# jyegerlehner/tensorflow-wavenet

Measured on AMD Instinct MI355X. Metric: audio samples/sec (train, default wavenet_params.json), higher is better.
Workload: dtype f32

## Files before the change

tensorflow-wavenet_amd/csrc/wn_gemm.hip:

```cpp
#include "wn_common.h"
#include <cstdlib>
#include <cstddef>
#include <cstring>

struct GemmNN {
  const float* A;
  long lda;
  long a_plane_stride;
  int a_planes;
  const float* W;
  int ldw;
  const float* bias;
  const float* mask;
  long ld_mask;
  const float* addend;
  long ld_add;
  float* C;
  long ldc;
  long c_plane_stride;
  int c_planes;
  float* Cpre;
  long M;
  int N, K;
  int relu;
// ... 162 lines not shown
        v[q] = *reinterpret_cast<const f32x4*>(tile + row * EP_LD + cc);
        if (g.mask && ok)
          mk[q] = __builtin_bit_cast(f32x4, __builtin_amdgcn_raw_buffer_load_b128(rM, vM, it * sM, EP_LD_AUX));
        if (g.addend && ok)
          ad[q] = __builtin_bit_cast(f32x4, __builtin_amdgcn_raw_buffer_load_b128(rA, vA, it * sA, EP_LD_AUX));
      }
#pragma unroll
      for (int q = 0; q < 4; ++q) {
        const int it = bt * 4 + q, row = it * 4 + rr;
        if (!(ncol && row < nrows)) continue;
        f32x4 x = v[q] + bias4;
        if (g.Cpre)
          __builtin_amdgcn_raw_buffer_store_b128(__builtin_bit_cast(ep_u32x4, x), rP, vP, it * sP, EP_ST_AUX);
        if (g.relu) {
#pragma unroll
          for (int e = 0; e < 4; ++e) x[e] = fmaxf(x[e], 0.f);
        }
        if (g.mask) {
#pragma unroll
          for (int e = 0; e < 4; ++e) x[e] = mk[q][e] > 0.f ? x[e] : 0.f;
        }
        if (g.addend) x += ad[q];
        __builtin_amdgcn_raw_buffer_store_b128(__builtin_bit_cast(ep_u32x4, x), rC, vC, it * sC, EP_ST_AUX);
      }
    }
  }
  }
}

template <int WMT>
__global__ __launch_bounds__(WMT * 128) void gemm_nn_kernel(GemmNN g) {
  constexpr int TM = WMT * 64, NT = WMT * 128;
  constexpr int NA = TM * 8 / NT, NB = 1024 / NT;
  __shared__ __attribute__((aligned(16))) float smem[2 * TM * NN_KC + 2 * NN_KC * NN_TN];
  float (*As)[TM * NN_KC] = reinterpret_cast<float (*)[TM * NN_KC]>(smem);
  float (*Bs)[NN_KC * NN_TN] =
      reinterpret_cast<float (*)[NN_KC * NN_TN]>(smem + 2 * TM * NN_KC);
  static_assert(WMT * 2 * 32 * EP_LD <= 2 * TM * NN_KC + 2 * NN_KC * NN_TN, "epilogue LDS");
  const int tid = threadIdx.x, lane = tid & 63, wave = tid >> 6;
  const int j = lane & 31, h = lane >> 5;
  const int wm = wave % WMT, wn = wave / WMT;
  const int logical = xcd_remap(blockIdx.x, g.nwg);
  const int tile_n = logical % g.tiles_n;
  const long m0 = (long)(logical / g.tiles_n) * TM;
  const int n0 = tile_n * NN_TN;
  const int nk = (g.K + NN_KC - 1) / NN_KC;
  f32x4 ra[NA], rb[NB];
  const bool full_m = m0 + TM <= g.M, full_n = n0 + NN_TN <= g.N;
  auto gload = [&](int kc) {
    const bool full_k = (kc + 1) * NN_KC <= g.K;
    if (full_m && full_k) {
      const float* pa = g.a_planes
                            ? g.A + (long)kc * g.a_plane_stride + m0 * 32
                            : g.A + m0 * g.lda + kc * NN_KC;
      const long ld = g.a_planes ? 32 : g.lda;
#pragma unroll
      for (int i = 0; i < NA; ++i)
        ra[i] = *reinterpret_cast<const f32x4*>(
            pa + (long)((tid >> 3) + (NT / 8) * i) * ld + (tid & 7) * 4);
    } else {
#pragma unroll
      for (int i = 0; i < NA; ++i) {
        const int row = (tid >> 3) + (NT / 8) * i, ch = tid & 7;
        const long m = m0 + row;
        const int k = kc * NN_KC + ch * 4;
        f32x4 v = {0.f, 0.f, 0.f, 0.f};
        if (m < g.M && k < g.K) {
          const float* p = g.a_planes
                               ? g.A + (long)kc * g.a_plane_stride + m * 32 + ch * 4
                               : g.A + m * g.lda + k;
          v = *reinterpret_cast<const f32x4*>(p);
        }
        ra[i] = v;
      }
    }
    if (full_n && full_k) {
      const float* pb = g.W + (long)kc * NN_KC * g.ldw + n0;
#pragma unroll
      for (int i = 0; i < NB; ++i)
        rb[i] = *reinterpret_cast<const f32x4*>(
            pb + (long)((tid >> 5) + (NT / 32) * i) * g.ldw + (tid & 31) * 4);
    } else {
#pragma unroll
      for (int i = 0; i < NB; ++i) {
        const int kk = (tid >> 5) + (NT / 32) * i, c4 = tid & 31;
        const int k = kc * NN_KC + kk, n = n0 + c4 * 4;
        f32x4 v = {0.f, 0.f, 0.f, 0.f};
        if (k < g.K && n < g.N)
          v = *reinterpret_cast<const f32x4*>(g.W + (long)k * g.ldw + n);
        rb[i] = v;
      }
    }
  };
  auto sstore = [&](int buf) {
#pragma unroll
    for (int i = 0; i < NA; ++i) {
      const int row = (tid >> 3) + (NT / 8) * i, ch = tid & 7;
      const int sw = ch ^ ((row >> 1) & 7);
      *reinterpret_cast<f32x4*>(&As[buf][row * NN_KC + sw * 4]) = ra[i];
    }
#pragma unroll
    for (int i = 0; i < NB; ++i) {
      const int kk = (tid >> 5) + (NT / 32) * i, c4 = tid & 31;
      *reinterpret_cast<f32x4*>(&Bs[buf][kk * NN_TN + c4 * 4]) = rb[i];
    }
  };

  f32x16 acc[2][2];
#pragma unroll
  for (int a = 0; a < 2; ++a)
#pragma unroll
    for (int b = 0; b < 2; ++b) acc[a][b] = frag_zero();

  gload(0);
  sstore(0);
  __syncthreads();
  for (int kc = 0; kc < nk; ++kc) {
    const int buf = kc & 1;
    if (kc + 1 < nk) gload(kc + 1);
    f32x16 fa[2];
#pragma unroll
    for (int fm = 0; fm < 2; ++fm) {
      const int row = wm * 64 + fm * 32 + j;
#pragma unroll
      for (int q = 0; q < 4; ++q) {
        const int sw = (2 * q + h) ^ ((j >> 1) & 7);
        const f32x4 v =
            *reinterpret_cast<const f32x4*>(&As[buf][row * NN_KC + sw * 4]);
        fa[fm][4 * q + 0] = v[0];
        fa[fm][4 * q + 1] = v[1];
        fa[fm][4 * q + 2] = v[2];
        fa[fm][4 * q + 3] = v[3];
      }
    }
    const float* bl = &Bs[buf][4 * h * NN_TN + wn * 64 + j];
#pragma unroll
    for (int r = 0; r < 16; ++r) {
      const int ko = (8 * (r >> 2) + (r & 3)) * NN_TN;
      const float w0 = bl[ko], w1 = bl[ko + 32];
      acc[0][0] = __builtin_amdgcn_mfma_f32_32x32x2f32(w0, fa[0][r], acc[0][0], 0, 0, 0);
      acc[0][1] = __builtin_amdgcn_mfma_f32_32x32x2f32(w0, fa[1][r], acc[0][1], 0, 0, 0);
      acc[1][0] = __builtin_amdgcn_mfma_f32_32x32x2f32(w1, fa[0][r], acc[1][0], 0, 0, 0);
      acc[1][1] = __builtin_amdgcn_mfma_f32_32x32x2f32(w1, fa[1][r], acc[1][1], 0, 0, 0);
    }
    if (kc + 1 < nk) sstore(buf ^ 1);
    __syncthreads();
  }

  gemm_epilogue(g, acc, smem, m0, n0, wm, wn, wave, lane);
}

#define N3_KC 16
#define N3_STAGE (NN_TM * N3_KC + N3_KC * NN_TN)

typedef __bf16 bf16x8 __attribute__((ext_vector_type(8)));
typedef unsigned int u32x4 __attribute__((ext_vector_type(4)));

struct Split3 {
  bf16x8 p[3];
};

__device__ __forceinline__ Split3 split3(const float (&v)[8]) {
  unsigned int hi[8], mi[8], lo[8];
#pragma unroll
  for (int e = 0; e < 8; ++e) {
    const unsigned int u = __float_as_uint(v[e]) & 0xffff0000u;
    const float r = v[e] - __uint_as_float(u);
    const unsigned int m = __float_as_uint(r) & 0xffff0000u;
    const float r2 = r - __uint_as_float(m);
    hi[e] = u;
    mi[e] = m;
    lo[e] = __float_as_uint(r2);
  }
  Split3 s;
  u32x4 ph, pm, pl;
#pragma unroll
  for (int w = 0; w < 4; ++w) {
    ph[w] = __builtin_amdgcn_perm(hi[2 * w + 1], hi[2 * w], 0x07060302u);
    pm[w] = __builtin_amdgcn_perm(mi[2 * w + 1], mi[2 * w], 0x07060302u);
    pl[w] = __builtin_amdgcn_perm(lo[2 * w + 1], lo[2 * w], 0x07060302u);
  }
  s.p[0] = __builtin_bit_cast(bf16x8, ph);
  s.p[1] = __builtin_bit_cast(bf16x8, pm);
  s.p[2] = __builtin_bit_cast(bf16x8, pl);
  return s;
}

template <int NPROD>
__device__ __forceinline__ void mma_split(f32x16& acc, const Split3& a, const Split3& b) {
#define WN_MM(i, k) \
  acc = __builtin_amdgcn_mfma_f32_32x32x16_bf16(a.p[i], b.p[k], acc, 0, 0, 0)
  if (NPROD >= 9) { WN_MM(2, 2); WN_MM(1, 2); WN_MM(2, 1); }
  if (NPROD >= 6) { WN_MM(1, 1); WN_MM(0, 2); WN_MM(2, 0); }
  WN_MM(0, 1);
  WN_MM(1, 0);
  WN_MM(0, 0);
#undef WN_MM
}

template <bool STAMPS>
__device__ __forceinline__ void nn3_tile(const GemmNN& g, float* smem, int tile_n, long m0,
                                         long m_end, unsigned long long* dbg) {
#define NSTAMP(i) if (STAMPS && threadIdx.x == 0) dbg[i] = __builtin_amdgcn_s_memtime()
  const int tid = threadIdx.x, lane = tid & 63;
  const int wave = __builtin_amdgcn_readfirstlane(tid >> 6);
  const int j = lane & 31, h = lane >> 5;
  const int wm = wave & 1, wn = wave >> 1;
  const int n0 = tile_n * NN_TN;
  const int nk = g.K / N3_KC;
  const bool live = n0 + wn * 64 < g.N;

  const int a_slot = lane & 3;
  const int a_chunk = a_slot ^ ((lane >> 4) & 3);
  long am0 = m0 + 16 * wave + (lane >> 2), am1 = am0 + 64;
  am0 = am0 < g.M ? am0 : g.M - 1;
  am1 = am1 < g.M ? am1 : g.M - 1;
  const long lda = g.a_planes ? 32 : g.lda;
  const int va0 = (int)((am0 * lda + a_chunk * 4) * 4);
  const int va1 = (int)((am1 * lda + a_chunk * 4) * 4);
  int wcol = n0 + (lane & 31) * 4;
  wcol = wcol < g.N ? wcol : 0;
  const int vw0 = (int)(((long)(2 * wave + (lane >> 5)) * g.ldw + wcol) * 4);
  const int vw1 = vw0 + (int)(8L * g.ldw * 4);
  auto stage = [&](int kc, float* base) {
    const __amdgpu_buffer_rsrc_t rsA = ep_rsrc(
        g.A + (g.a_planes ? (long)(kc >> 1) * g.a_plane_stride + (kc & 1) * 16 : (long)kc * N3_KC));
    const __amdgpu_buffer_rsrc_t rsW = ep_rsrc(g.W + (long)kc * N3_KC * g.ldw);
    __builtin_amdgcn_raw_ptr_buffer_load_lds(rsA, (lptr_t)(base + wave * 256), 16, va0, 0, 0, 0);
    __builtin_amdgcn_raw_ptr_buffer_load_lds(rsA, (lptr_t)(base + (wave + 4) * 256), 16, va1, 0, 0, 0);
    float* wb = base + NN_TM * N3_KC;
    __builtin_amdgcn_raw_ptr_buffer_load_lds(rsW, (lptr_t)(wb + wave * 256), 16, vw0, 0, 0, 0);
    __builtin_amdgcn_raw_ptr_buffer_load_lds(rsW, (lptr_t)(wb + (wave + 4) * 256), 16, vw1, 0, 0, 0);
  };

  f32x16 acc[2][2];
#pragma unroll
  for (int a = 0; a < 2; ++a)
#pragma unroll
    for (int b = 0; b < 2; ++b) acc[a][b] = frag_zero();

  stage(0, smem);
  if (!live) {
    for (int kc = 0; kc < nk; ++kc) {
      asm volatile("s_waitcnt vmcnt(0)\n\ts_barrier" ::: "memory");
      if (kc + 1 < nk) stage(kc + 1, smem + ((kc & 1) ^ 1) * N3_STAGE);
    }
  }
  for (int kc = 0; live && kc < nk; ++kc) {
    const int ST = kc & 1;
    asm volatile("s_waitcnt vmcnt(0)\n\ts_barrier" ::: "memory");
    if (STAMPS && kc == 0) { NSTAMP(1); }
    if (kc + 1 < nk) stage(kc + 1, smem + (ST ^ 1) * N3_STAGE);
    const float* As = smem + ST * N3_STAGE;
    const float* Bs = As + NN_TM * N3_KC;
    f32x4 fa[2][2];
#pragma unroll
    for (int fm = 0; fm < 2; ++fm) {
      const int row = wm * 64 + fm * 32 + j;
#pragma unroll
      for (int q = 0; q < 2; ++q)
        fa[fm][q] = *reinterpret_cast<const f32x4*>(
            As + row * N3_KC + (((2 * q + h) ^ ((row >> 2) & 3)) << 2));
    }
    const float* bl = Bs + 4 * h * NN_TN + wn * 64 + j;
    __builtin_amdgcn_s_setprio(1);
    constexpr int PF = NN3_PF;
    float wv[8][2];
#pragma unroll
    for (int r = 0; r < PF; ++r) {
      const int ko = (8 * (r >> 2) + (r & 3)) * NN_TN;
      wv[r][0] = bl[ko];
      wv[r][1] = bl[ko + 32];
    }
    __builtin_amdgcn_sched_barrier(0);
#pragma unroll
    for (int r = 0; r < 8; ++r) {
      if (r + PF < 8) {
        const int ko = (8 * ((r + PF) >> 2) + ((r + PF) & 3)) * NN_TN;
        wv[r + PF][0] = bl[ko];
        wv[r + PF][1] = bl[ko + 32];
      }
      __builtin_amdgcn_sched_barrier(0);
      const float w0 = wv[r][0], w1 = wv[r][1];
      const float x0 = fa[0][r >> 2][r & 3], x1 = fa[1][r >> 2][r & 3];
      acc[0][0] = __builtin_amdgcn_mfma_f32_32x32x2f32(w0, x0, acc[0][0], 0, 0, 0);
      acc[0][1] = __builtin_amdgcn_mfma_f32_32x32x2f32(w0, x1, acc[0][1], 0, 0, 0);
      acc[1][0] = __builtin_amdgcn_mfma_f32_32x32x2f32(w1, x0, acc[1][0], 0, 0, 0);
      acc[1][1] = __builtin_amdgcn_mfma_f32_32x32x2f32(w1, x1, acc[1][1], 0, 0, 0);
      __builtin_amdgcn_sched_barrier(0);
    }
    __builtin_amdgcn_s_setprio(0);
  }
  NSTAMP(2);
  asm volatile("s_waitcnt lgkmcnt(0)\n\ts_barrier" ::: "memory");
  NSTAMP(3);
  gemm_epilogue(g, acc, smem, m0, n0, wm, wn, wave, lane, m_end);
  NSTAMP(4);
#undef NSTAMP
}

constexpr int NN3_LDSF = 2 * N3_STAGE > 4 * 32 * EP_LD ? 2 * N3_STAGE : 4 * 32 * EP_LD;

__global__ __launch_bounds__(256, 4) void gemm_nn3_kernel(GemmNN g) {
  __shared__ __attribute__((aligned(1024))) float smem[NN3_LDSF];
  unsigned long long* dbg = nullptr;
#ifdef NN3_STAMPS
// ... 341 lines not shown
  __shared__ __attribute__((aligned(16))) float As[32 * TM];
  __shared__ __attribute__((aligned(16))) float Gs[32 * TNW];
  const int tid = threadIdx.x, lane = tid & 63, wave = tid >> 6;
  const int i = lane & 31, h = lane >> 5;
  const int tn = blockIdx.x % g.tiles_n, tm = blockIdx.x / g.tiles_n;
  const int m0 = tm * TM, n0 = tn * TNW;
  const long r_begin = (long)blockIdx.y * g.rows_per_split;
  long r_end = r_begin + g.rows_per_split;
  if (r_end > g.rows) r_end = g.rows;

  f32x16 acc[MF][NF];
#pragma unroll
  for (int a = 0; a < MF; ++a)
#pragma unroll
    for (int b = 0; b < NF; ++b) acc[a][b] = frag_zero();
  float cs[NF];
#pragma unroll
  for (int b = 0; b < NF; ++b) cs[b] = 0.f;

  f32x4 ra[NA], rg[NG];
  auto gload = [&](long r0) {
#pragma unroll
    for (int k = 0; k < NA; ++k) {
      const int idx = tid + 256 * k;
      f32x4 v = {0.f, 0.f, 0.f, 0.f};
      if (idx < 32 * A4) {
        const int row = idx / A4, c4 = idx - row * A4;
        const long r = r0 + row;
        if (r < r_end) {
          const int m = m0 + c4 * 4;
          const float* p = g.a_planes
                               ? g.A + (long)(m >> 5) * g.a_plane_stride + r * 32 + (m & 31)
                               : g.A + r * g.lda + m;
          v = *reinterpret_cast<const f32x4*>(p);
        }
      }
      ra[k] = v;
    }
#pragma unroll
    for (int k = 0; k < NG; ++k) {
      const int idx = tid + 256 * k;
      const int row = idx / G4, c4 = idx - row * G4;
      const long r = r0 + row;
      f32x4 v = {0.f, 0.f, 0.f, 0.f};
      if (r < r_end)
        v = *reinterpret_cast<const f32x4*>(g.G + r * g.ldg + n0 + c4 * 4);
      rg[k] = v;
    }
  };
  auto sstore = [&]() {
#pragma unroll
    for (int k = 0; k < NA; ++k) {
      const int idx = tid + 256 * k;
      if (idx < 32 * A4) *reinterpret_cast<f32x4*>(&As[idx * 4]) = ra[k];
    }
#pragma unroll
    for (int k = 0; k < NG; ++k)
      *reinterpret_cast<f32x4*>(&Gs[(tid + 256 * k) * 4]) = rg[k];
  };

  gload(r_begin);
  sstore();
  __syncthreads();
  for (long r0 = r_begin; r0 < r_end; r0 += 32) {
    const bool more = r0 + 32 < r_end;
    if (more) gload(r0 + 32);
    const float* al = As + h * TM + i;
    const float* gl = Gs + h * TNW + wave * (NF * 32) + i;
#pragma unroll 2
    for (int s = 0; s < 16; ++s) {
      float av[MF], bv[NF];
#pragma unroll
      for (int a = 0; a < MF; ++a) av[a] = al[2 * s * TM + a * 32];
#pragma unroll
      for (int b = 0; b < NF; ++b) {
        bv[b] = gl[2 * s * TNW + b * 32];
        cs[b] += bv[b];
      }
#pragma unroll
      for (int a = 0; a < MF; ++a)
#pragma unroll
        for (int b = 0; b < NF; ++b)
          acc[a][b] = __builtin_amdgcn_mfma_f32_32x32x2f32(av[a], bv[b], acc[a][b], 0, 0, 0);
    }
    __syncthreads();
    if (more) sstore();
    __syncthreads();
  }

  float* slab = g.slabs + (long)blockIdx.y * g.slab_stride;
#pragma unroll
  for (int a = 0; a < MF; ++a)
#pragma unroll
    for (int b = 0; b < NF; ++b) {
      const int n = n0 + wave * (NF * 32) + b * 32 + i;
#pragma unroll
      for (int rr = 0; rr < 16; ++rr) {
        const int m = m0 + a * 32 + 8 * (rr >> 2) + 4 * h + (rr & 3);
        slab[(long)m * g.Nw + n] = acc[a][b][rr];
      }
    }
  if (g.want_colsum && (tm == 0 || g.want_colsum == 2)) {
#pragma unroll
    for (int b = 0; b < NF; ++b) {
      float v = cs[b] + __shfl_xor(cs[b], 32);
      const int n = n0 + wave * (NF * 32) + b * 32 + i;
      if (h == 0) slab[(long)g.Mw * g.Nw + (long)tm * g.Nw + n] = tm == 0 ? v : 0.f;
    }
  }
}

typedef float f32x2 __attribute__((ext_vector_type(2)));
struct wn_true { static constexpr bool value = true; };
struct wn_false { static constexpr bool value = false; };
template <int MF, int NF>
__global__ __launch_bounds__(256, (MF * NF >= 10 ? 2 : MF * NF > 5 ? 3 : 4)) void gemm_tn3_kernel(GemmTN g) {
  constexpr int TM = MF * 32, TNW = 4 * NF * 32, KR = 16;
  constexpr int STAGE = KR * TM + KR * TNW;
  constexpr int PA = KR * TM / 256, PG = KR * TNW / 256;
  __shared__ __attribute__((aligned(1024))) float smem[2 * STAGE];
  const int tid = threadIdx.x, lane = tid & 63;
  const int wave = __builtin_amdgcn_readfirstlane(tid >> 6);
  const int i = lane & 31, h = lane >> 5;
  const int ntile = gridDim.x;
  const int logical = xcd_remap(blockIdx.x + ntile * blockIdx.y, ntile * gridDim.y);
  const int tile = logical % ntile, split = logical / ntile;
  const int tn = tile % g.tiles_n, tm = tile / g.tiles_n;
  const int m0 = tm * TM, n0 = tn * TNW;
  const long r_begin = (long)split * g.rows_per_split;
  long r_end = r_begin + g.rows_per_split;
  if (r_end > g.rows) r_end = g.rows;
  const int nchunks = r_end > r_begin ? (int)((r_end - r_begin + KR - 1) / KR) : 0;
  const int tail_rows = nchunks ? (int)(r_end - r_begin) - (nchunks - 1) * KR : KR;

  constexpr int NPA = (PA + 3) / 4, NPG = (PG + 3) / 4;
  const long rowA = g.a_planes ? 32 * 4 : g.lda * 4, rowG = g.ldg * 4;
  const __amdgpu_buffer_rsrc_t rsA = ep_rsrc(
      g.a_planes ? g.A + (long)(m0 >> 5) * g.a_plane_stride + r_begin * 32
                 : g.A + r_begin * g.lda + m0);
  const __amdgpu_buffer_rsrc_t rsG = ep_rsrc(g.G + r_begin * g.ldg + n0);
  int voA[3], voG[4];
  static_assert(NPA <= 3 && NPG <= 4, "pieces per wave");
#pragma unroll
  for (int k = 0; k < NPA; ++k) {
    const int e = (wave + 4 * k) * 256 + lane * 4;
    const int row = e / TM, col = e - row * TM;
    voA[k] = g.a_planes ? (int)(((long)(col >> 5) * g.a_plane_stride + row * 32 + (col & 31)) * 4)
                        : (int)(((long)row * g.lda + col) * 4);
  }
#pragma unroll
  for (int k = 0; k < NPG; ++k) {
    const int e = (wave + 4 * k) * 256 + lane * 4;
    const int row = e / TNW, col = e - row * TNW;
    voG[k] = (int)(((long)row * g.ldg + col) * 4);
  }
  auto stage = [&](int c, int st) {
    float* base = smem + st * STAGE;
    const long r0 = (long)c * KR;
    const unsigned sA = (unsigned)(r0 * rowA), sG = (unsigned)(r0 * rowG);
    float* gb = base + KR * TM;
    if (tail_rows < KR && c == nchunks - 1) {
      const f32x4 zero = {0.f, 0.f, 0.f, 0.f};
#pragma unroll
      for (int k = 0; k < NPA; ++k)
        if (wave + 4 * k < PA)
          *reinterpret_cast<f32x4*>(base + (wave + 4 * k) * 256 + lane * 4) = zero;
#pragma unroll
      for (int k = 0; k < NPG; ++k)
        if (wave + 4 * k < PG)
          *reinterpret_cast<f32x4*>(gb + (wave + 4 * k) * 256 + lane * 4) = zero;
      asm volatile("s_waitcnt lgkmcnt(0)" ::: "memory");
#pragma unroll
      for (int k = 0; k < NPA; ++k) {
        const int p = wave + 4 * k;
        if (p < PA && (p * 256 + lane * 4) / TM < tail_rows)
          __builtin_amdgcn_raw_ptr_buffer_load_lds(rsA, (lptr_t)(base + p * 256), 16, voA[k], sA, 0, 0);
      }
#pragma unroll
      for (int k = 0; k < NPG; ++k) {
        const int p = wave + 4 * k;
        if (p < PG && (p * 256 + lane * 4) / TNW < tail_rows)
          __builtin_amdgcn_raw_ptr_buffer_load_lds(rsG, (lptr_t)(gb + p * 256), 16, voG[k], sG, 0, 0);
      }
      return;
    }
#pragma unroll
    for (int k = 0; k < NPA; ++k) {
      const int p = wave + 4 * k;
      if (p < PA)
        __builtin_amdgcn_raw_ptr_buffer_load_lds(rsA, (lptr_t)(base + p * 256), 16, voA[k], sA, 0, 0);
    }
#pragma unroll
    for (int k = 0; k < NPG; ++k) {
      const int p = wave + 4 * k;
      if (p < PG)
        __builtin_amdgcn_raw_ptr_buffer_load_lds(rsG, (lptr_t)(gb + p * 256), 16, voG[k], sG, 0, 0);
    }
  };

  f32x16 acc[MF][NF];
#pragma unroll
  for (int a = 0; a < MF; ++a)
#pragma unroll
    for (int b = 0; b < NF; ++b) acc[a][b] = frag_zero();
  float cs[NF];
  f32x2 cs2[NF];
#pragma unroll
  for (int b = 0; b < NF; ++b) {
    cs[b] = 0.f;
    cs2[b] = f32x2{0.f, 0.f};
  }

  if (nchunks > 0) stage(0, 0);
  auto kloop = [&](auto cs_tag, int c_begin, int c_end) {
    constexpr bool SUM = decltype(cs_tag)::value;
    for (int c = c_begin; c < c_end; ++c) {
      const int st = c & 1;
      asm volatile("s_waitcnt vmcnt(0)\n\ts_barrier" ::: "memory");
      if (c + 1 < nchunks) stage(c + 1, st ^ 1);
      const float* al = smem + st * STAGE + h * TM + i;
      const float* gl = smem + st * STAGE + KR * TM + h * TNW + wave * (NF * 32) + i;
      __builtin_amdgcn_s_setprio(1);
      if (SUM && MF * NF == 8) {
#pragma unroll
        for (int s2 = 0; s2 < KR / 2; ++s2) {
          float a_[MF], b_[NF];
#pragma unroll
          for (int a = 0; a < MF; ++a) a_[a] = al[2 * s2 * TM + a * 32];
#pragma unroll
          for (int b = 0; b < NF; ++b) {
            b_[b] = gl[2 * s2 * TNW + b * 32];
            cs[b] += b_[b];
          }
#pragma unroll
          for (int a = 0; a < MF; ++a)
#pragma unroll
            for (int b = 0; b < NF; ++b)
              acc[a][b] = __builtin_amdgcn_mfma_f32_32x32x2f32(a_[a], b_[b], acc[a][b], 0, 0, 0);
        }
        __builtin_amdgcn_s_setprio(0);
        continue;
      }
      float av[2][MF], bv[2][NF], keep[KR / 2][NF];
      static_assert(KR == 16, "column-sum tree");
      auto fetch = [&](int s2, float (&a_)[MF], float (&b_)[NF]) {
#pragma unroll
        for (int a = 0; a < MF; ++a) a_[a] = al[2 * s2 * TM + a * 32];
#pragma unroll
        for (int b = 0; b < NF; ++b) b_[b] = gl[2 * s2 * TNW + b * 32];
      };
      fetch(0, av[0], bv[0]);
      __builtin_amdgcn_sched_barrier(0);
#pragma unroll
      for (int s2 = 0; s2 < KR / 2; ++s2) {
        if (s2 + 1 < KR / 2) fetch(s2 + 1, av[(s2 + 1) & 1], bv[(s2 + 1) & 1]);
        __builtin_amdgcn_sched_barrier(0);
#pragma unroll
        for (int a = 0; a < MF; ++a)
#pragma unroll
          for (int b = 0; b < NF; ++b)
            acc[a][b] = __builtin_amdgcn_mfma_f32_32x32x2f32(av[s2 & 1][a], bv[s2 & 1][b],
                                                             acc[a][b], 0, 0, 0);
        if (SUM) {
#pragma unroll
          for (int b = 0; b < NF; ++b) keep[s2][b] = bv[s2 & 1][b];
        }
        __builtin_amdgcn_sched_barrier(0);
      }
      if (SUM) {
#pragma unroll
        for (int b = 0; b < NF; ++b) {
          const f32x2 p0 = {keep[0][b], keep[1][b]}, p1 = {keep[2][b], keep[3][b]};
          const f32x2 p2 = {keep[4][b], keep[5][b]}, p3 = {keep[6][b], keep[7][b]};
          cs2[b] += (p0 + p1) + (p2 + p3);
        }
      }
      __builtin_amdgcn_s_setprio(0);
    }
  };
  const bool spread = g.want_colsum == 2;
  const bool do_cs = spread ? true : (g.want_colsum && tm == (split + 3 * tn) % g.tiles_m);
  if (spread) {
    const int own = (tm + split + 3 * tn) % g.tiles_m;
    for (int c0 = 0; c0 < nchunks; c0 += g.tiles_m) {
      const int ce = min(nchunks, c0 + g.tiles_m);
      const int cs_at = min(ce, c0 + own);
      kloop(wn_false{}, c0, cs_at);
      kloop(wn_true{}, cs_at, min(ce, cs_at + 1));
      kloop(wn_false{}, min(ce, cs_at + 1), ce);
    }
  } else if (do_cs) {
    kloop(wn_true{}, 0, nchunks);
  } else {
    kloop(wn_false{}, 0, nchunks);
  }

  float* slab = g.slabs + (long)split * g.slab_stride;
#pragma unroll
  for (int a = 0; a < MF; ++a)
#pragma unroll
    for (int b = 0; b < NF; ++b) {
      const int n = n0 + wave * (NF * 32) + b * 32 + i;
#pragma unroll
      for (int rr = 0; rr < 16; ++rr) {
        const int m = m0 + a * 32 + 8 * (rr >> 2) + 4 * h + (rr & 3);
        __builtin_nontemporal_store(acc[a][b][rr], slab + (long)m * g.Nw + n);
      }
    }
  if (do_cs) {
#pragma unroll
    for (int b = 0; b < NF; ++b) {
      cs[b] += cs2[b].x + cs2[b].y;
      float v = cs[b] + __shfl_xor(cs[b], 32);
      const int n = n0 + wave * (NF * 32) + b * 32 + i;
      if (h == 0) slab[(long)g.Mw * g.Nw + (spread ? (long)tm * g.Nw : 0) + n] = v;
    }
  }
}

template <int NPROD>
__global__ __launch_bounds__(256, 3) void gemm_tn_split_kernel(GemmTN g) {
  constexpr int KR = 16, TT = 128;
  constexpr int STAGE = 2 * KR * TT;
  __shared__ __attribute__((aligned(1024))) float smem[2 * STAGE];
  const int tid = threadIdx.x, lane = tid & 63;
  const int wave = __builtin_amdgcn_readfirstlane(tid >> 6);
  const int i = lane & 31, h = lane >> 5;
  const int wm = wave & 1, wn = wave >> 1;
  const int ntile = gridDim.x;
  const int logical = xcd_remap(blockIdx.x + ntile * blockIdx.y, ntile * gridDim.y);
  const int tile = logical % ntile, split = logical / ntile;
  const int tn = tile % g.tiles_n, tm = tile / g.tiles_n;
  const int m0 = tm * TT, n0 = tn * TT;
  const long r_begin = (long)split * g.rows_per_split;
  long r_end = r_begin + g.rows_per_split;
  if (r_end > g.rows) r_end = g.rows;
  const int nchunks = r_end > r_begin ? (int)((r_end - r_begin) / KR) : 0;

  const int prow = lane >> 5, pcol = (lane & 31) * 4;
  int am = m0 + pcol;
  am = am < g.Mw ? am : g.Mw - 4;
  int gn = n0 + pcol;
  gn = gn < g.Nw ? gn : g.Nw - 4;
  auto stage = [&](int c, int st) {
    float* base = smem + st * STAGE;
    const long r0 = r_begin + (long)c * KR;
#pragma unroll
    for (int q = 0; q < 2; ++q) {
      const int p = wave + 4 * q;
      const long row = r0 + 2 * p + prow;
      const float* src = g.a_planes
                             ? g.A + (long)(am >> 5) * g.a_plane_stride + row * 32 + (am & 31)
                             : g.A + row * g.lda + am;
      __builtin_amdgcn_global_load_lds((gptr_t)src, (lptr_t)(base + p * 256), 16, 0, 0);
      __builtin_amdgcn_global_load_lds((gptr_t)(g.G + row * g.ldg + gn),
                                       (lptr_t)(base + KR * TT + p * 256), 16, 0, 0);
    }
  };

  f32x16 acc[2][2];
#pragma unroll
  for (int a = 0; a < 2; ++a)
#pragma unroll
    for (int b = 0; b < 2; ++b) acc[a][b] = frag_zero();
  float cs[2] = {0.f, 0.f};

  if (nchunks > 0) stage(0, 0);
  for (int c = 0; c < nchunks; ++c) {
    const int st = c & 1;
    asm volatile("s_waitcnt vmcnt(0)\n\ts_barrier" ::: "memory");
    if (c + 1 < nchunks) stage(c + 1, st ^ 1);
    const float* al = smem + st * STAGE + 8 * h * TT + wm * 64 + i;
    const float* gl = smem + st * STAGE + KR * TT + 8 * h * TT + wn * 64 + i;
    Split3 as[2], gs[2];
#pragma unroll
    for (int f = 0; f < 2; ++f) {
      float v[8];
#pragma unroll
      for (int e = 0; e < 8; ++e) v[e] = al[e * TT + f * 32];
      as[f] = split3(v);
    }
#pragma unroll
    for (int f = 0; f < 2; ++f) {
      float v[8];
#pragma unroll
      for (int e = 0; e < 8; ++e) {
        v[e] = gl[e * TT + f * 32];
        cs[f] += v[e];
      }
      gs[f] = split3(v);
    }
#pragma unroll
    for (int a = 0; a < 2; ++a)
#pragma unroll
      for (int b = 0; b < 2; ++b) mma_split<NPROD>(acc[a][b], as[a], gs[b]);
  }

  float* slab = g.slabs + (long)split * g.slab_stride;
#pragma unroll
  for (int a = 0; a < 2; ++a)
#pragma unroll
    for (int b = 0; b < 2; ++b) {
      const int n = n0 + wn * 64 + b * 32 + i;
      if (n >= g.Nw) continue;
#pragma unroll
      for (int rr = 0; rr < 16; ++rr) {
        const int m = m0 + wm * 64 + a * 32 + 8 * (rr >> 2) + 4 * h + (rr & 3);
        if (m < g.Mw) slab[(long)m * g.Nw + n] = acc[a][b][rr];
      }
    }
  if (g.want_colsum && tm == 0 && wm == 0) {
#pragma unroll
    for (int b = 0; b < 2; ++b) {
      const float v = cs[b] + __shfl_xor(cs[b], 32);
      const int n = n0 + wn * 64 + b * 32 + i;
      if (h == 0 && n < g.Nw) slab[(long)g.Mw * g.Nw + n] = v;
    }
  }
}

__global__ void reduce_slabs_kernel(const float* __restrict__ slabs,
                                    int num_slabs, long slab_stride,
                                    long in_batch_stride, long offset, long n,
                                    float* __restrict__ dst,
                                    long out_batch_stride, int replicate,
                                    long rep_stride) {
  const long e = (long)blockIdx.x * blockDim.x + threadIdx.x;
  if (e >= n) return;
  const int b = blockIdx.y;
  const float* p = slabs + (long)b * in_batch_stride + offset + e;
  float s0 = 0.f, s1 = 0.f, s2 = 0.f, s3 = 0.f;
  int s = 0;
  for (; s + 3 < num_slabs; s += 4) {
    s0 += p[(long)s * slab_stride];
    s1 += p[(long)(s + 1) * slab_stride];
    s2 += p[(long)(s + 2) * slab_stride];
    s3 += p[(long)(s + 3) * slab_stride];
  }
  for (; s < num_slabs; ++s) s0 += p[(long)s * slab_stride];
  const float v = (s0 + s1) + (s2 + s3);
  for (int r = 0; r < replicate; ++r)
    dst[(long)b * out_batch_stride + (long)r * rep_stride + e] = v;
}

template <int PARTS>
__global__ void reduce_slabs4_kernel(const float* __restrict__ slabs,
                                     int num_slabs, long slab_stride,
// ... 574 lines not shown
```

Measured before the change: 13.26 million.

## Unroll weight-grad k-loop by stage parity and permute G columns in LDS

The split-K weight-gradient kernel's chunk loop is restructured so the double-buffer stage index is a compile-time constant, unrolling chunks in pairs. LDS read addresses are precomputed once and hidden behind an empty asm, so every fragment load can use an immediate offset instead of per-chunk address arithmetic. The G-tile global-to-LDS mapping is permuted so each wave's fragments are interleaved with a 128-float stride. The spread column-sum schedule is also flattened into a single loop. This targets VALU/SALU address overhead in the MFMA inner loop, at the cost of larger code and a more intricate column mapping that must stay consistent with the epilogue.

Result: slower. 12.96 million (-2.3%).

```diff
diff --git a/tensorflow-wavenet_amd/csrc/wn_gemm.hip b/tensorflow-wavenet_amd/csrc/wn_gemm.hip
--- a/tensorflow-wavenet_amd/csrc/wn_gemm.hip
+++ b/tensorflow-wavenet_amd/csrc/wn_gemm.hip
@@ -338,6 +338,7 @@
 
 #define N3_KC 16
 #define N3_STAGE (NN_TM * N3_KC + N3_KC * NN_TN)
+template <int V> struct wn_int { static constexpr int value = V; };
 
 typedef __bf16 bf16x8 __attribute__((ext_vector_type(8)));
 typedef unsigned int u32x4 __attribute__((ext_vector_type(4)));
@@ -985,7 +986,8 @@
   for (int k = 0; k < NPG; ++k) {
     const int e = (wave + 4 * k) * 256 + lane * 4;
     const int row = e / TNW, col = e - row * TNW;
-    voG[k] = (int)(((long)row * g.ldg + col) * 4);
+    const int gcol = ((col & 127) >> 5) * (NF * 32) + (col >> 7) * 32 + (col & 31);
+    voG[k] = (int)(((long)row * g.ldg + gcol) * 4);
   }
   auto stage = [&](int c, int st) {
     float* base = smem + st * STAGE;
@@ -1045,24 +1047,33 @@
   }
 
   if (nchunks > 0) stage(0, 0);
-  auto kloop = [&](auto cs_tag, int c_begin, int c_end) {
+  int oal0 = (h * TM + i) * 4, oal1 = oal0 + 32 * 4;
+  int ogl = (KR * TM + h * TNW + wave * 32 + i) * 4;
+  asm volatile("" : "+v"(oal0), "+v"(oal1), "+v"(ogl));
+  const char* smem_b = reinterpret_cast<const char*>(smem);
+  const float* al0 = reinterpret_cast<const float*>(smem_b + oal0);
+  const float* al1 = reinterpret_cast<const float*>(smem_b + oal1);
+  const float* gl0 = reinterpret_cast<const float*>(smem_b + ogl);
+  auto chunk = [&](auto cs_tag, auto st_tag, int c) __attribute__((always_inline)) {
     constexpr bool SUM = decltype(cs_tag)::value;
-    for (int c = c_begin; c < c_end; ++c) {
-      const int st = c & 1;
+    constexpr int st = decltype(st_tag)::value;
+    {
       asm volatile("s_waitcnt vmcnt(0)\n\ts_barrier" ::: "memory");
       if (c + 1 < nchunks) stage(c + 1, st ^ 1);
-      const float* al = smem + st * STAGE + h * TM + i;
-      const float* gl = smem + st * STAGE + KR * TM + h * TNW + wave * (NF * 32) + i;
+      auto rdA = [&](int s2, int a) {
+        return ((a & 1) ? al1 : al0)[st * STAGE + 2 * s2 * TM + (a >> 1) * 64];
+      };
+      auto rdG = [&](int s2, int b) { return gl0[st * STAGE + 2 * s2 * TNW + b * 128]; };
       __builtin_amdgcn_s_setprio(1);
       if (SUM && MF * NF == 8) {
 #pragma unroll
         for (int s2 = 0; s2 < KR / 2; ++s2) {
           float a_[MF], b_[NF];
 #pragma unroll
-          for (int a = 0; a < MF; ++a) a_[a] = al[2 * s2 * TM + a * 32];
+          for (int a = 0; a < MF; ++a) a_[a] = rdA(s2, a);
 #pragma unroll
           for (int b = 0; b < NF; ++b) {
-            b_[b] = gl[2 * s2 * TNW + b * 32];
+            b_[b] = rdG(s2, b);
             cs[b] += b_[b];
           }
 #pragma unroll
@@ -1072,15 +1083,15 @@
               acc[a][b] = __builtin_amdgcn_mfma_f32_32x32x2f32(a_[a], b_[b], acc[a][b], 0, 0, 0);
         }
         __builtin_amdgcn_s_setprio(0);
-        continue;
+        return;
       }
       float av[2][MF], bv[2][NF], keep[KR / 2][NF];
       static_assert(KR == 16, "column-sum tree");
       auto fetch = [&](int s2, float (&a_)[MF], float (&b_)[NF]) {
 #pragma unroll
-        for (int a = 0; a < MF; ++a) a_[a] = al[2 * s2 * TM + a * 32];
-#pragma unroll
-        for (int b = 0; b < NF; ++b) b_[b] = gl[2 * s2 * TNW + b * 32];
+        for (int a = 0; a < MF; ++a) a_[a] = rdA(s2, a);
+#pragma unroll
+        for (int b = 0; b < NF; ++b) b_[b] = rdG(s2, b);
       };
       fetch(0, av[0], bv[0]);
       __builtin_amdgcn_sched_barrier(0);
@@ -1111,21 +1122,27 @@
       __builtin_amdgcn_s_setprio(0);
     }
   };
+  auto kloop = [&](auto cs_tag, int c_begin, int c_end) __attribute__((always_inline)) {
+    int c = c_begin;
+    if (c < c_end && (c & 1)) chunk(cs_tag, wn_int<1>{}, c++);
+    for (; c + 1 < c_end; c += 2) {
+      chunk(cs_tag, wn_int<0>{}, c);
+      chunk(cs_tag, wn_int<1>{}, c + 1);
+    }
+    if (c < c_end) chunk(cs_tag, wn_int<0>{}, c);
+  };
   const bool spread = g.want_colsum == 2;
   const bool do_cs = spread ? true : (g.want_colsum && tm == (split + 3 * tn) % g.tiles_m);
-  if (spread) {
-    const int own = (tm + split + 3 * tn) % g.tiles_m;
-    for (int c0 = 0; c0 < nchunks; c0 += g.tiles_m) {
-      const int ce = min(nchunks, c0 + g.tiles_m);
-      const int cs_at = min(ce, c0 + own);
-      kloop(wn_false{}, c0, cs_at);
-      kloop(wn_true{}, cs_at, min(ce, cs_at + 1));
-      kloop(wn_false{}, min(ce, cs_at + 1), ce);
-    }
-  } else if (do_cs) {
+  if (!spread && do_cs) {
     kloop(wn_true{}, 0, nchunks);
   } else {
-    kloop(wn_false{}, 0, nchunks);
+    int cs_at = spread ? (tm + split + 3 * tn) % g.tiles_m : nchunks;
+    for (int c = 0; c < nchunks; cs_at += g.tiles_m) {
+      const int ce = min(nchunks, cs_at);
+      kloop(wn_false{}, c, ce);
+      kloop(wn_true{}, ce, min(nchunks, ce + 1));
+      c = ce + 1;
+    }
   }
 
   float* slab = g.slabs + (long)split * g.slab_stride;
```
